# gpustack/llama-box

Measured on AMD Instinct MI355X. Metric: decode tokens/sec (batch-1) + prefill tok/s, Llama-3-8B Q4_K_M, higher is better.
Workload: dtype q4_K/q6_K weights x q8_K activations (int8 dot, f32 accumulate)

## Files before the change

### llama_box_amd/csrc/fattn.hip

```cpp
#include <algorithm>

#include "dev_util.h"
#include "kernels.h"
#include <vector>
#include <algorithm>
#include "kv_dequant.h"

namespace mi355x {

static inline bool fa_g_ok(const int64_t G) {
    static const int g_min = getenv("GGML_MI355X_FA_G_MIN") ? atoi(getenv("GGML_MI355X_FA_G_MIN")) : 1;
    return G >= g_min && G <= 8;
}
static inline int fa_gg(const int64_t G) { return G <= 2 ? 2 : (G <= 4 ? 4 : 8); }

thread_local int g_fa_form = 0;
static inline void fa_form_tail(int tail) { g_fa_form = (g_fa_form & ~(7 << 13)) | (tail << 13); }

struct fa_geom {
    int n_q, n_head, n_kv_head, n_kv, n_splits, has_mask;
    int rec_stride;
    float scale, softcap, max_bias, m0, m1;
    uint32_t n_head_log2;
    unsigned * arrive;
// ... 6 lines not shown
__device__ __forceinline__ float xrow_allsum(const float x) {
    float a = x, b = x;
    asm volatile("s_nop 1\n\tv_permlane16_swap_b32 %0, %1" : "+v"(a), "+v"(b));
    float y = a + b;
    a = y;
    b = y;
    asm volatile("s_nop 1\n\tv_permlane32_swap_b32 %0, %1" : "+v"(a), "+v"(b));
    return a + b;
}

template <int D, int G>
__global__ void __launch_bounds__(256) k_fattn_split(const tdesc q, const tdesc k, const tdesc v, const tdesc mask, const float * __restrict__ sinks,
                                                     const tdesc dst, const fa_geom geo, float * __restrict__ ws) {
    constexpr int LPR = D / 8;
    constexpr int RPW = 64 / LPR;
    constexpr int NG = 4;
    __shared__ float sh[4][G][D + 2];
    const int tid = threadIdx.x, lane = tid & 63, wave = tid >> 6;
    const int sub = lane / LPR, sl = lane % LPR;
    const int split = blockIdx.x, kvh = blockIdx.y;
    const int tok = blockIdx.z % geo.n_q, bat = blockIdx.z / geo.n_q;
    const int per = (geo.n_kv + geo.n_splits - 1) / geo.n_splits;
    const int kv0 = split * per, kv1 = min(geo.n_kv, kv0 + per);
    const int64_t kb = bat / (q.ne[3] / k.ne[3]), vb = bat / (q.ne[3] / v.ne[3]);
    const uint16_t * mp = geo.has_mask ? (const uint16_t *) (mask.data + (int64_t) tok * mask.nb[1] + (int64_t) (bat % mask.ne[3]) * mask.nb[3]) : nullptr;
    const char * kbase = k.data + (int64_t) kvh * k.nb[2] + kb * k.nb[3] + sl * 16;
    const char * vbase = v.data + (int64_t) kvh * v.nb[2] + vb * v.nb[3] + sl * 16;

    uint4 kraw[NG], vraw[NG];
    float mv[NG];
    bool inr[NG];
    int p0 = kv0 + wave * RPW;
#define FA_LOAD_TRIP()                                                        \
    _Pragma("unroll") for (int u = 0; u < NG; ++u) {                         \
        const int p = p0 + u * 4 * RPW + sub;                                 \
        inr[u] = p < kv1;                                                     \
        const int pc = min(p, kv1 - 1);                                       \
        mv[u] = mp ? h2f(mp[pc]) : 0.0f;                                      \
        kraw[u] = *(const uint4 *) (kbase + (int64_t) pc * k.nb[1]);          \
        vraw[u] = *(const uint4 *) (vbase + (int64_t) pc * v.nb[1]);          \
    }
    if (kv0 < kv1) { FA_LOAD_TRIP() }

    float qr[G][8], acc[G][8], m[G], l[G], slope[G];
#pragma unroll
    for (int g = 0; g < G; ++g) {
        const int h = kvh * G + g;
        const float4 * qp = (const float4 *) ((const float *) (q.data + (int64_t) tok * q.nb[1] + (int64_t) h * q.nb[2] + (int64_t) bat * q.nb[3]) + sl * 8);
        const float4 qa = qp[0], qb = qp[1];
        const float qv[8] = {qa.x, qa.y, qa.z, qa.w, qb.x, qb.y, qb.z, qb.w};
#pragma unroll
        for (int i = 0; i < 8; ++i) {
            qr[g][i] = h2f(f2h(qv[i]));
            acc[g][i] = 0.0f;
        }
        m[g] = -INFINITY;
        l[g] = 0.0f;
        slope[g] = geo.max_bias > 0.0f ? ((uint32_t) h < geo.n_head_log2 ? powf(geo.m0, (float) (h + 1)) : powf(geo.m1, (float) (2 * (h - geo.n_head_log2) + 1))) : 1.0f;
    }

    for (; p0 < kv1; p0 += NG * 4 * RPW) {
        float sc[NG][G];
        float vf[NG][8];
#pragma unroll
        for (int u = 0; u < NG; ++u) {
            const uint32_t ku[4] = {kraw[u].x, kraw[u].y, kraw[u].z, kraw[u].w}, vu[4] = {vraw[u].x, vraw[u].y, vraw[u].z, vraw[u].w};
            float kf[8];
#pragma unroll
            for (int i = 0; i < 4; ++i) {
                kf[2 * i] = h2f((uint16_t) (ku[i] & 0xFFFF));
                kf[2 * i + 1] = h2f((uint16_t) (ku[i] >> 16));
                vf[u][2 * i] = h2f((uint16_t) (vu[i] & 0xFFFF));
                vf[u][2 * i + 1] = h2f((uint16_t) (vu[i] >> 16));
            }
#pragma unroll
            for (int g = 0; g < G; ++g) {
                float t = 0.0f;
#pragma unroll
                for (int i = 0; i < 8; ++i) t = fmaf(kf[i], qr[g][i], t);
                if constexpr (LPR == 16) {
                    t = row16_sum(t);
                } else {
                    t += dpp_f32<MI_DPP_QUAD_XOR1>(t);
                    t += dpp_f32<MI_DPP_QUAD_XOR2>(t);
                    t += dpp_f32<MI_DPP_HALF_MIRROR>(t);
                }
                float sv = t * geo.scale;
                if (geo.softcap != 0.0f) sv = geo.softcap * tanhf(sv);
                const float mvs = slope[g] * mv[u];
                sv += mvs;
                sc[u][g] = (inr[u] && !(mvs == -INFINITY)) ? sv : -INFINITY;
            }
        }
        const bool more = p0 + NG * 4 * RPW < kv1;
        if (more) {
            p0 += NG * 4 * RPW;
            FA_LOAD_TRIP()
            p0 -= NG * 4 * RPW;
        }
#pragma unroll
        for (int g = 0; g < G; ++g) {
            float mx = sc[0][g];
#pragma unroll
            for (int u = 1; u < NG; ++u) mx = fmaxf(mx, sc[u][g]);
            mx = wave_max(mx);
            const float mn = fmaxf(m[g], mx);
            if (mn == -INFINITY) continue;
            const float alpha = m[g] == -INFINITY ? 0.0f : expf(m[g] - mn);
            float ps = 0.0f;
#pragma unroll
            for (int i = 0; i < 8; ++i) acc[g][i] *= alpha;
#pragma unroll
            for (int u = 0; u < NG; ++u) {
                const float pe = sc[u][g] == -INFINITY ? 0.0f : expf(sc[u][g] - mn);
                ps += pe;
#pragma unroll
                for (int i = 0; i < 8; ++i) acc[g][i] = fmaf(pe, vf[u][i], acc[g][i]);
            }
            l[g] = l[g] * alpha + ps;
            m[g] = mn;
        }
    }
#undef FA_LOAD_TRIP
#pragma unroll
    for (int g = 0; g < G; ++g) {
        float lt = l[g];
        if constexpr (LPR == 8) lt += dpp_f32<MI_DPP_ROR8>(lt);
        lt = xrow_allsum(lt);
#pragma unroll
        for (int i = 0; i < 8; ++i) {
            float a = acc[g][i];
            if constexpr (LPR == 8) a += dpp_f32<MI_DPP_ROR8>(a);
            acc[g][i] = xrow_allsum(a);
        }
        l[g] = lt;
    }
    if (sub == 0) {
#pragma unroll
        for (int g = 0; g < G; ++g) {
            *(float4 *) &sh[wave][g][sl * 8] = make_float4(acc[g][0], acc[g][1], acc[g][2], acc[g][3]);
            *(float4 *) &sh[wave][g][sl * 8 + 4] = make_float4(acc[g][4], acc[g][5], acc[g][6], acc[g][7]);
            if (sl == 0) {
                sh[wave][g][D] = m[g];
                sh[wave][g][D + 1] = l[g];
            }
        }
    }
    __syncthreads();
    for (int e = tid; e < G * D; e += 256) {
        const int g = e / D, dd = e % D;
        const float m0 = sh[0][g][D], m1 = sh[1][g][D], m2 = sh[2][g][D], m3 = sh[3][g][D];
        const float mt = fmaxf(fmaxf(m0, m1), fmaxf(m2, m3));
        const float c0 = m0 == -INFINITY ? 0.0f : expf(m0 - mt), c1 = m1 == -INFINITY ? 0.0f : expf(m1 - mt);
        const float c2 = m2 == -INFINITY ? 0.0f : expf(m2 - mt), c3 = m3 == -INFINITY ? 0.0f : expf(m3 - mt);
        float a = ((sh[0][g][dd] * c0 + sh[1][g][dd] * c1) + sh[2][g][dd] * c2) + sh[3][g][dd] * c3;
        float lt = ((sh[0][g][D + 1] * c0 + sh[1][g][D + 1] * c1) + sh[2][g][D + 1] * c2) + sh[3][g][D + 1] * c3;
        const int h = kvh * G + g;
        if (geo.n_splits == 1) {
            if (sinks) {
                const float sk = sinks[h];
                const float mn = fmaxf(mt, sk);
                const float c = mt == -INFINITY ? 0.0f : expf(mt - mn);
                a *= c;
                lt = lt * c + expf(sk - mn);
            }
            float * out = (float *) (dst.data + (int64_t) h * dst.nb[1] + (int64_t) tok * dst.nb[2] + (int64_t) bat * dst.nb[3]);
            out[dd] = a * (1.0f / lt);
        } else {
            float * rec = ws + ((((int64_t) bat * geo.n_q + tok) * geo.n_head + h) * geo.n_splits + split) * (D + 2);
            rec[dd] = a;
            if (dd == 0) {
                rec[D] = mt;
                rec[D + 1] = lt;
            }
        }
    }
}

#define MI_DPP_NEWBCAST(n) (0x150 + (n))
typedef _Float16 fa_half2 __attribute__((ext_vector_type(2)));

__device__ __forceinline__ float fa_exp2(const float x) { return __builtin_amdgcn_exp2f(x); }
__device__ __forceinline__ float swap32_pairsum(float x, float y) {
    asm volatile("s_nop 1\n\tv_permlane32_swap_b32 %0, %1" : "+v"(x), "+v"(y));
    return x + y;
}
__device__ __forceinline__ float swap16_pairsum(float c, float d) {
    asm volatile("s_nop 1\n\tv_permlane16_swap_b32 %0, %1" : "+v"(c), "+v"(d));
    return c + d;
}
__device__ __forceinline__ float xrow_allmax(const float x) {
    float a = x, b = x;
    asm volatile("s_nop 1\n\tv_permlane16_swap_b32 %0, %1" : "+v"(a), "+v"(b));
    const float y = fmaxf(a, b);
    a = y;
    b = y;
    asm volatile("s_nop 1\n\tv_permlane32_swap_b32 %0, %1" : "+v"(a), "+v"(b));
    return fmaxf(a, b);
}
__device__ __forceinline__ void st_agent(float * p, const float v) { __hip_atomic_store(p, v, __ATOMIC_RELAXED, __HIP_MEMORY_SCOPE_AGENT); }
__device__ __forceinline__ float ld_agent(const float * p) { return __hip_atomic_load(p, __ATOMIC_RELAXED, __HIP_MEMORY_SCOPE_AGENT); }
__device__ __forceinline__ void st_agent2(float * p, const float a, const float b) {
    const unsigned long long v = (unsigned long long) __builtin_bit_cast(unsigned, a) | ((unsigned long long) __builtin_bit_cast(unsigned, b) << 32);
    __hip_atomic_store((unsigned long long *) p, v, __ATOMIC_RELAXED, __HIP_MEMORY_SCOPE_AGENT);
}
__device__ __forceinline__ float2 ld_agent2(const float * p) {
    const unsigned long long v = __hip_atomic_load((const unsigned long long *) p, __ATOMIC_RELAXED, __HIP_MEMORY_SCOPE_AGENT);
    return make_float2(__builtin_bit_cast(float, (unsigned) v), __builtin_bit_cast(float, (unsigned) (v >> 32)));
}
#define FA_M2_REC 132

__device__ __forceinline__ void fa_merge2(const float * __restrict__ hb, const int h0, const int g_real, const int n_splits, const float * __restrict__ sinks, const tdesc & dst,
                                          const int tok, const int bat, const int n_threads) {
    const int tid = threadIdx.x, lane = tid & 63;
    const int64_t ss = (int64_t) g_real * FA_M2_REC;
#pragma unroll 1
    for (int g = tid >> 7; g < g_real; g += n_threads >> 7) {
        const int dd = tid & 127;
        const float * __restrict__ base = hb + (int64_t) g * FA_M2_REC;
        const float2 ml = ld_agent2(base + (int64_t) min(lane, n_splits - 1) * ss + 128);
        float r[32];
#pragma unroll
        for (int u = 0; u < 32; ++u) r[u] = ld_agent(base + (int64_t) min(u, n_splits - 1) * ss + dd);
        const float ms = lane < n_splits ? ml.x : -INFINITY, ls = lane < n_splits ? ml.y : 0.0f;
        float mn = wave_max(ms);
        float sink_term = 0.0f;
        if (sinks) {
            mn = fmaxf(mn, sinks[h0 + g]);
            sink_term = expf(sinks[h0 + g] - mn);
        }
        const float cs = ms == -INFINITY ? 0.0f : expf(ms - mn);
        const float lt = wave_sum(ls * cs) + sink_term;
        float a = 0.0f;
#pragma unroll
        for (int u = 0; u < 32; ++u) {
            const float c = readlane_f32(cs, u);
            a += c != 0.0f ? r[u] * c : 0.0f;
        }
        float * out = (float *) (dst.data + (int64_t) (h0 + g) * dst.nb[1] + (int64_t) tok * dst.nb[2] + (int64_t) bat * dst.nb[3]);
        out[dd] = a * (1.0f / lt);
    }
}

__device__ __forceinline__ void fa_merge_heads(const float * __restrict__ base0, const int h0, const int g_real, const int n_splits, const float * __restrict__ sinks, const tdesc & dst,
                                               const int tok, const int bat, q8k_dev * __restrict__ q8, float * __restrict__ vals) {
    constexpr int D = 128;
    const int tid = threadIdx.x, lane = tid & 63, wave = tid >> 6;
    if (q8) __syncthreads();
    for (int g = wave; g < g_real; g += 4) {
        const float * __restrict__ base = base0 + (int64_t) g * n_splits * (D + 2);
        const bool has = lane < n_splits;
        const float ms = has ? ld_agent(base + (int64_t) lane * (D + 2) + D) : -INFINITY;
        const float ls = has ? ld_agent(base + (int64_t) lane * (D + 2) + D + 1) : 0.0f;
        float mn = wave_max(ms);
        float sink_term = 0.0f;
        if (sinks) {
            mn = fmaxf(mn, sinks[h0 + g]);
            sink_term = expf(sinks[h0 + g] - mn);
        }
        const float cs = ms == -INFINITY ? 0.0f : expf(ms - mn);
        const float lt = wave_sum(ls * cs) + sink_term;
        float a0 = 0.0f, a1 = 0.0f;
        for (int u0 = 0; u0 < n_splits; u0 += 8) {
            float r0[8], r1[8];
#pragma unroll
            for (int k = 0; k < 8; ++k) {
                const int u = min(u0 + k, n_splits - 1);
                r0[k] = ld_agent(base + (int64_t) u * (D + 2) + lane);
                r1[k] = ld_agent(base + (int64_t) u * (D + 2) + 64 + lane);
            }
#pragma unroll
            for (int k = 0; k < 8; ++k) {
                const float c = u0 + k < n_splits ? readlane_f32(cs, min(u0 + k, 63)) : 0.0f;
                a0 += c != 0.0f ? r0[k] * c : 0.0f;
                a1 += c != 0.0f ? r1[k] * c : 0.0f;
            }
        }
        const float inv = 1.0f / lt;
        if (q8) {
            vals[g * D + lane] = a0 * inv;
            vals[g * D + 64 + lane] = a1 * inv;
        } else {
            float * out = (float *) (dst.data + (int64_t) (h0 + g) * dst.nb[1] + (int64_t) tok * dst.nb[2] + (int64_t) bat * dst.nb[3]);
            out[lane] = a0 * inv;
            out[64 + lane] = a1 * inv;
        }
    }
    if (q8) {
        __syncthreads();
        if (wave < g_real / 2) {
            const float4 t4 = ((const float4 *) (vals + wave * 256))[lane];
            const float t[4] = {t4.x, t4.y, t4.z, t4.w};
            wave_quantize_q8_K(t, lane, q8 + wave);
        }
    }
}

#ifdef FA_STAMP
__device__ unsigned long long g_fa_stamps[1024][8];
#define FA_STAMP_AT(i) { if (WV == 8 && MODE == 0 && threadIdx.x == 0) g_fa_stamps[(blockIdx.y * gridDim.x + blockIdx.x) & 1023][(i)] = __builtin_readcyclecounter(); }
#else
#define FA_STAMP_AT(i)
#endif
template <int G, int MODE, bool Q8, int WV = 4, int KVT = 0, int D = 128>
__global__ void __launch_bounds__(WV * 64) k_fattn_dec128(const tdesc q, const tdesc k, const tdesc v, const tdesc mask, const float * __restrict__ sinks,
                                                      const tdesc dst, const fa_geom geo, float * __restrict__ ws, const int g_real,
                                                      const int * __restrict__ lists, const int list_stride) {
    constexpr bool SKIP = MODE == 1, LIST = MODE == 2;
    constexpr int LPR = D / 8, RPW = 64 / LPR, NG = LPR / G;
    static_assert(D == 128 || (D == 64 && !Q8 && KVT == 0 && G <= 8), "head_dim 64: f16 cache only");
    constexpr float LOG2E = 1.4426950408889634f;
    constexpr int TRIP = NG * WV * RPW;
    constexpr bool BF = KVT == GGML_TYPE_BF16;
    constexpr bool DQ = KVT != 0 && !BF;
    static_assert(WV == 4 || (!Q8 && !DQ && !BF), "the eight-wave forms serve an f16 cache only");
    static_assert(!(Q8 && DQ), "q8_0 has its own integer path");
    constexpr bool FAT = WV == 8 && MODE == 0;
    FA_STAMP_AT(0)
    __shared__ float sh[WV][G][D + 2];
    __shared__ float qv[FAT ? 1 : G * D];
    const int tid = threadIdx.x, lane = tid & 63, wave = tid >> 6;
    const int sub = lane / LPR, sl = lane & (LPR - 1);
    const int ul = sl / G, gl = sl % G;
    const int split = blockIdx.x, kvh = blockIdx.y;
    const int tok = (int) blockIdx.z;
    constexpr int bat = 0;
    const int per = geo.per;
    const int kv0 = LIST ? 0 : min(split * per, geo.n_kv);
    int kv1 = LIST ? 0 : min(geo.n_kv, kv0 + per);
    const int * tl = nullptr;
    int ti = 0, ti1 = 0, cnt = 0;
    bool empty = false;
    int nidx[NG];
    int first = 0;
#define FA_LIST_AHEAD(base)                                                                                         \
    _Pragma("unroll") for (int u = 0; u < NG; ++u) nidx[u] = tl[min((base) + u * (WV * RPW) + wave * RPW + sub, geo.n_kv - 1)];
    if constexpr (LIST) {
        const int * lt = lists + (int64_t) tok * list_stride;
        tl = lt + 1;
        cnt = lt[0];
        first = lt[1];
        if (geo.n_splits == 1) FA_LIST_AHEAD(0)
        const int trips = (cnt + TRIP - 1) / TRIP, share = (trips + geo.n_splits - 1) / geo.n_splits;
        ti = split * share;
        ti1 = min(trips, ti + share);
        if (ti >= ti1) {
            if (geo.n_splits == 1) {
                for (int e = tid; e < g_real * D; e += WV * 64) {
                    float * out = (float *) (dst.data + (int64_t) (kvh * g_real + e / D) * dst.nb[1] + (int64_t) tok * dst.nb[2] + (int64_t) bat * dst.nb[3]);
                    out[e % D] = __builtin_nanf("");
                }
            } else if (tid < g_real) {
                float * rec = ws + ((((int64_t) bat * geo.n_q + tok) * geo.n_head + kvh * g_real + tid) * geo.n_splits + split) * (D + 2);
                if (geo.arrive) { st_agent(rec + D, -INFINITY); st_agent(rec + D + 1, 0.0f); }
                else { rec[D] = -INFINITY; rec[D + 1] = 0.0f; }
            }
            if (geo.n_splits == 1 || !geo.arrive) return;
            empty = true;
        }
        kv1 = cnt;
        if (geo.n_splits != 1 && !empty) FA_LIST_AHEAD(ti * TRIP)
    }
    constexpr int64_t kb = 0, vb = 0, mb = 0;
    if constexpr (SKIP) {
        const uint16_t * mrow = (const uint16_t *) (mask.data + (int64_t) tok * mask.nb[1] + mb * mask.nb[3]);
        bool any = false;
        for (int c0 = kv0; c0 < kv1; c0 += 256) {
            const int pp = c0 + 4 * lane;
            if (pp < kv1) {
                const uint2 w = *(const uint2 *) (mrow + pp);
                any = any || w.x != 0xFC00FC00u || w.y != 0xFC00FC00u;
            }
        }
        if (!__any(any)) {
            if (tid < g_real) {
                float * rec = ws + ((((int64_t) bat * geo.n_q + tok) * geo.n_head + kvh * g_real + tid) * geo.n_splits + split) * (D + 2);
                if (geo.arrive) { st_agent(rec + D, -INFINITY); st_agent(rec + D + 1, 0.0f); }
                else { rec[D] = -INFINITY; rec[D + 1] = 0.0f; }
            }
            if (!geo.arrive) return;
            empty = true;
        }
    }
    if (!empty) {
    const uint16_t * mp = geo.has_mask ? (const uint16_t *) (mask.data + (int64_t) tok * mask.nb[1] + mb * mask.nb[3]) : nullptr;
    const char * kbase = k.data + (int64_t) kvh * k.nb[2] + kb * k.nb[3] + (DQ ? (sl >> 2) * kv_block_bytes_t<KVT>() : Q8 ? (sl >> 2) * 34 + 2 + (sl & 3) * 8 : sl * 16);
    const char * vbase = v.data + (int64_t) kvh * v.nb[2] + vb * v.nb[3] + (DQ ? (sl >> 2) * kv_block_bytes_t<KVT>() : Q8 ? (sl >> 2) * 34 + 2 + (sl & 3) * 8 : sl * 16);

    uint4 kraw[NG], vraw[NG];
    float mvl = 0.0f;
    bool okl = false;
    int p0 = LIST ? ti * TRIP : kv0;
#define FA_LOAD_TRIP()                                                                  \
    {                                                                                   \
        _Pragma("unroll") for (int u = 0; u < NG; ++u) {                               \
            const int pr_ = p0 + u * (WV * RPW) + wave * RPW + sub;                     \
            const int pc = LIST ? (pr_ < kv1 ? nidx[u] : first) : min(pr_, kv1 - 1);    \
            const char * kp_ = kbase + (int64_t) pc * k.nb[1];                          \
            const char * vp_ = vbase + (int64_t) pc * v.nb[1];                          \
            if constexpr (DQ) {   \
                kraw[u] = kv_load_octet_raw_t<KVT>(kp_, sl & 3);                        \
                vraw[u] = kv_load_octet_raw_t<KVT>(vp_, sl & 3);                        \
            } else if constexpr (Q8) {    \
                kraw[u] = make_uint4(ld32_a2(kp_), ld32_a2(kp_ + 4), (uint32_t) ld16(kp_ - 2 - (sl & 3) * 8), 0u);  \
                vraw[u] = make_uint4(ld32_a2(vp_), ld32_a2(vp_ + 4), (uint32_t) ld16(vp_ - 2 - (sl & 3) * 8), 0u);  \
            } else {                                                                    \
                kraw[u] = *(const uint4 *) kp_;                                         \
                vraw[u] = *(const uint4 *) vp_;                                         \
            }                                                                           \
        }                                                                               \
        const int pl = p0 + ul * (WV * RPW) + wave * RPW + sub;                         \
        okl = pl < kv1;                                                                 \
        int plc_ = min(pl, kv1 - 1);                                                    \
        if constexpr (LIST) {                                                           \
            plc_ = nidx[0];                                                             \
            _Pragma("unroll") for (int u = 1; u < NG; ++u) plc_ = ul == u ? nidx[u] : plc_; \
            plc_ = okl ? plc_ : first;                                                  \
        }                                                                               \
        mvl = mp ? h2f(mp[plc_]) : 0.0f;                                                \
        if constexpr (LIST) FA_LIST_AHEAD(p0 + TRIP)                                    \
    }
    uint32_t vis = 0xFFFFFFFFu;
    if constexpr (SKIP) {
        vis = 0;
        const int ntrips = (kv1 - kv0 + TRIP - 1) / TRIP;
        for (int i0 = 0; i0 < ntrips; i0 += 8) {
            uint16_t mraw[8];
#pragma unroll
            for (int i = 0; i < 8; ++i) {
                const int pl = kv0 + (i0 + i) * TRIP + ul * (WV * RPW) + wave * RPW + sub;
                mraw[i] = (i0 + i < ntrips && pl < kv1) ? (mp ? mp[pl] : (uint16_t) 0) : (uint16_t) 0xFC00;
            }
#pragma unroll
            for (int i = 0; i < 8; ++i)
                if (__any(mraw[i] != 0xFC00)) vis |= 1u << (i0 + i);
        }
        if (vis & 1u) FA_LOAD_TRIP()
    } else {
        if (kv0 < kv1) FA_LOAD_TRIP()
    }
    FA_STAMP_AT(1)

    fa_half2 qh[G][4];
    int qq[G][2];
    float dq[G];
    int qsb[G];
    float sq[G];
    float qf[BF ? G : 1][8];
#pragma unroll
    for (int g = 0; g < G; ++g) {
        const int h = kvh * g_real + min(g, g_real - 1);
        const float4 * qp = (const float4 *) ((const float *) (q.data + (int64_t) tok * q.nb[1] + (int64_t) h * q.nb[2] + (int64_t) bat * q.nb[3]) + sl * 8);
        const float4 qa = qp[0], qb = qp[1];
        const float z = g < g_real ? 1.0f : 0.0f;
        if constexpr (BF) {
            const float xv[8] = {qa.x * z, qa.y * z, qa.z * z, qa.w * z, qb.x * z, qb.y * z, qb.z * z, qb.w * z};
#pragma unroll
            for (int i = 0; i < 8; ++i) {
                const uint32_t u = __float_as_uint(xv[i]);
                qf[g][i] = __uint_as_float((u + (0x7fffu + ((u >> 16) & 1u))) & 0xffff0000u);
            }
        } else if constexpr (Q8 || DQ) {
            const float xv[8] = {qa.x * z, qa.y * z, qa.z * z, qa.w * z, qb.x * z, qb.y * z, qb.z * z, qb.w * z};
            float amax = 0.0f;
#pragma unroll
            for (int i = 0; i < 8; ++i) amax = fmaxf(amax, fabsf(xv[i]));
            amax = fmaxf(amax, dpp_f32<MI_DPP_QUAD_XOR1>(amax));
            amax = fmaxf(amax, dpp_f32<MI_DPP_QUAD_XOR2>(amax));
            const float d = amax / 127.0f;
            const float id = d != 0.0f ? 1.0f / d : 0.0f;
            uint32_t w0 = 0, w1 = 0;
#pragma unroll
            for (int i = 0; i < 4; ++i) {
                w0 |= (uint32_t) ((int) roundf(xv[i] * id) & 0xFF) << (8 * i);
                w1 |= (uint32_t) ((int) roundf(xv[4 + i] * id) & 0xFF) << (8 * i);
            }
            qq[g][0] = (int) w0;
            qq[g][1] = (int) w1;
            dq[g] = h2f(f2h(d));
            if constexpr (DQ) {
                int qs_ = dot4((int) w0, 0x01010101, dot4((int) w1, 0x01010101, 0));
                qs_ += dpp_i32<MI_DPP_QUAD_XOR1>(qs_);
                qs_ += dpp_i32<MI_DPP_QUAD_XOR2>(qs_);
                qsb[g] = qs_;
                sq[g] = h2f(f2h((float) qs_ * d));
            }
        } else {
            qh[g][0] = (fa_half2){(_Float16) (qa.x * z), (_Float16) (qa.y * z)};
            qh[g][1] = (fa_half2){(_Float16) (qa.z * z), (_Float16) (qa.w * z)};
            qh[g][2] = (fa_half2){(_Float16) (qb.x * z), (_Float16) (qb.y * z)};
            qh[g][3] = (fa_half2){(_Float16) (qb.z * z), (_Float16) (qb.w * z)};
        }
    }
#ifdef FA_STAMP
    asm volatile("s_waitcnt vmcnt(8)" ::: "memory");
    FA_STAMP_AT(2)
#endif
    float acc[G][8];
#pragma unroll
    for (int g = 0; g < G; ++g)
#pragma unroll
        for (int i = 0; i < 8; ++i) acc[g][i] = 0.0f;
    float m = -INFINITY, l = 0.0f;
    const bool b3 = (sl & 8) != 0, b2 = (sl & 4) != 0, b1 = (sl & 2) != 0, b0 = (sl & 1) != 0;
    const float sc2 = geo.scale * LOG2E;

    for (int trip = 0; LIST ? ti < ti1 : p0 < kv1; ++trip) {
        int p_next = p0 + TRIP;
        if constexpr (LIST) {
            ++ti;
            p_next = ti < ti1 ? ti * TRIP : kv1;
        }
        if constexpr (SKIP) {
            if (!((vis >> trip) & 1u)) {
                if (p_next < kv1 && ((vis >> (trip + 1)) & 1u)) {
                    p0 = p_next;
                    FA_LOAD_TRIP()
                }
                p0 = p_next;
                continue;
            }
        }
        float t[LPR];
        float vf[NG][8];
#pragma unroll
        for (int u = 0; u < NG; ++u) {
            uint32_t ku[4] = {kraw[u].x, kraw[u].y, kraw[u].z, kraw[u].w}, vu[4] = {vraw[u].x, vraw[u].y, vraw[u].z, vraw[u].w};
            if constexpr (DQ) {
                constexpr bool OFFSET = KVT == GGML_TYPE_Q4_1 || KVT == GGML_TYPE_Q5_1;
                uint32_t k0, k1;
                kv_octet_levels_t<KVT, true>(kraw[u], sl & 3, k0, k1);
                const float dk = h2f((uint16_t) (ku[2] & 0xFFFFu));
                const float mk = OFFSET ? h2f((uint16_t) (ku[2] >> 16)) : 0.0f;
                kv_octet_f32_t<KVT>(vraw[u], sl & 3, vf[u]);
#pragma unroll
                for (int g = 0; g < G; ++g) {
                    int isum = dot4((int) k0, qq[g][0], dot4((int) k1, qq[g][1], 0));
                    isum += dpp_i32<MI_DPP_QUAD_XOR1>(isum);
                    isum += dpp_i32<MI_DPP_QUAD_XOR2>(isum);
                    float term;
                    if constexpr (KVT == GGML_TYPE_Q4_0) term = ((float) (isum - 8 * qsb[g]) * dk) * dq[g];
                    else if constexpr (KVT == GGML_TYPE_Q5_0) term = (dk * dq[g]) * (float) (isum - 16 * qsb[g]);
                    else if constexpr (KVT == GGML_TYPE_IQ4_NL) term = (dq[g] * dk) * (float) isum;
                    else term = (dk * dq[g]) * (float) isum + mk * sq[g];
                    t[u * G + g] = (sl & 3) == 0 ? term : 0.0f;
                }
            } else if constexpr (Q8) {
                const float dv = h2f((uint16_t) vu[2]), dk = h2f((uint16_t) ku[2]);
#pragma unroll
                for (int i = 0; i < 4; ++i) {
                    vf[u][i] = (float) (int) (int8_t) (vu[0] >> (8 * i)) * dv;
                    vf[u][4 + i] = (float) (int) (int8_t) (vu[1] >> (8 * i)) * dv;
                }
#pragma unroll
                for (int g = 0; g < G; ++g) {
                    int isum = dot4((int) ku[0], qq[g][0], dot4((int) ku[1], qq[g][1], 0));
                    isum += dpp_i32<MI_DPP_QUAD_XOR1>(isum);
                    isum += dpp_i32<MI_DPP_QUAD_XOR2>(isum);
                    t[u * G + g] = (sl & 3) == 0 ? (float) isum * (dk * dq[g]) : 0.0f;
                }
            } else if constexpr (BF) {
                float kf_[8];
#pragma unroll
                for (int i = 0; i < 4; ++i) {
                    vf[u][2 * i] = __uint_as_float(vu[i] << 16);
                    vf[u][2 * i + 1] = __uint_as_float(vu[i] & 0xffff0000u);
                    kf_[2 * i] = __uint_as_float(ku[i] << 16);
                    kf_[2 * i + 1] = __uint_as_float(ku[i] & 0xffff0000u);
                }
#pragma unroll
                for (int g = 0; g < G; ++g) {
                    float d = 0.0f;
#pragma unroll
                    for (int i = 0; i < 8; ++i) d = __builtin_fmaf(kf_[i], qf[g][i], d);
                    t[u * G + g] = d;
                }
            } else {
#pragma unroll
                for (int i = 0; i < 4; ++i) {
                    vf[u][2 * i] = h2f((uint16_t) (vu[i] & 0xFFFF));
                    vf[u][2 * i + 1] = h2f((uint16_t) (vu[i] >> 16));
                }
#pragma unroll
                for (int g = 0; g < G; ++g) {
                    float d = 0.0f;
#pragma unroll
                    for (int i = 0; i < 4; ++i) d = __builtin_amdgcn_fdot2(__builtin_bit_cast(fa_half2, ku[i]), qh[g][i], d, false);
                    t[u * G + g] = d;
                }
            }
        }
#ifdef FA_STAMP
        if (trip == 0) { asm volatile("" :: "v"(t[0]), "v"(t[15])); FA_STAMP_AT(3) }
#endif
        const bool more = p_next < kv1 && (!SKIP || ((vis >> (trip + 1)) & 1u));
        const float mv_cur = mvl;
        const bool ok_cur = okl;
        p0 = p_next;
        if (more) FA_LOAD_TRIP()
        float w8[8], w4[4], w2[2];
#pragma unroll
        for (int j = 0; j < 8; ++j) {
            if constexpr (LPR == 16) {
                const float keep = b3 ? t[j + 8] : t[j], send = b3 ? t[j] : t[j + 8];
                w8[j] = keep + dpp_f32<MI_DPP_ROR8>(send);
            } else {
                w8[j] = t[j];
            }
        }
#pragma unroll
        for (int j = 0; j < 4; ++j) {
            const float keep = b2 ? w8[j + 4] : w8[j], send = b2 ? w8[j] : w8[j + 4];
            w4[j] = keep + dpp_f32<MI_DPP_HALF_MIRROR>(send);
        }
#pragma unroll
        for (int j = 0; j < 2; ++j) {
            const float keep = b1 ? w4[j + 2] : w4[j], send = b1 ? w4[j] : w4[j + 2];
            w2[j] = keep + dpp_f32<MI_DPP_QUAD_XOR2>(send);
        }
        float sv;
        {
            const float keep = b0 ? w2[1] : w2[0], send = b0 ? w2[0] : w2[1];
            sv = keep + dpp_f32<MI_DPP_QUAD_XOR1>(send);
        }
        sv = (ok_cur && !(mv_cur == -INFINITY)) ? fmaf(sv, sc2, mv_cur * LOG2E) : -INFINITY;
        float mx = sv;
        if constexpr (G <= 2) mx = fmaxf(mx, dpp_f32<MI_DPP_ROR2>(mx));
        if constexpr (G <= 4) mx = fmaxf(mx, dpp_f32<MI_DPP_ROR4>(mx));
        mx = fmaxf(mx, dpp_f32<MI_DPP_ROR8>(mx));
        mx = xrow_allmax(mx);
        const float mn = fmaxf(m, mx);
        const float mref = mn == -INFINITY ? 0.0f : mn;
        const float alpha = fa_exp2(m - mref);
        const float pe = fa_exp2(sv - mref);
        l = l * alpha + pe;
        m = mn;
#define FA_HEAD(g)                                                                          \
    if constexpr ((g) < G) {                                                                \
        const float ag_ = dpp_f32<MI_DPP_NEWBCAST((g))>(alpha);                             \
        _Pragma("unroll") for (int i = 0; i < 8; ++i) acc[(g)][i] *= ag_;                  \
    }
        FA_HEAD(0) FA_HEAD(1) FA_HEAD(2) FA_HEAD(3) FA_HEAD(4) FA_HEAD(5) FA_HEAD(6) FA_HEAD(7)
#undef FA_HEAD
#define FA_PAIR(j)                                                                          \
    {                                                                                       \
        const float pj_ = dpp_f32<MI_DPP_NEWBCAST((j))>(pe);                                \
        _Pragma("unroll") for (int i = 0; i < 8; ++i) acc[(j) % G][i] = fmaf(pj_, vf[(j) / G][i], acc[(j) % G][i]); \
    }
#define FA_PAIR8(j)                                                                         \
    {                                                                                       \
        const float pa_ = dpp_f32<MI_DPP_NEWBCAST((j))>(pe), pb_ = dpp_f32<MI_DPP_NEWBCAST((j) + 8)>(pe); \
        const float pj_ = (lane & 8) ? pb_ : pa_;                                           \
        _Pragma("unroll") for (int i = 0; i < 8; ++i) acc[(j) % G][i] = fmaf(pj_, vf[(j) / G][i], acc[(j) % G][i]); \
    }
        if constexpr (LPR == 16) {
            FA_PAIR(0) FA_PAIR(1) FA_PAIR(2) FA_PAIR(3) FA_PAIR(4) FA_PAIR(5) FA_PAIR(6) FA_PAIR(7)
            FA_PAIR(8) FA_PAIR(9) FA_PAIR(10) FA_PAIR(11) FA_PAIR(12) FA_PAIR(13) FA_PAIR(14) FA_PAIR(15)
        } else {
            FA_PAIR8(0) FA_PAIR8(1) FA_PAIR8(2) FA_PAIR8(3) FA_PAIR8(4) FA_PAIR8(5) FA_PAIR8(6) FA_PAIR8(7)
        }
#undef FA_PAIR8
#undef FA_PAIR
    }
#undef FA_LOAD_TRIP
#undef FA_LIST_AHEAD
#ifdef FA_STAMP
    asm volatile("" :: "v"(acc[0][0]), "v"(acc[G - 1][7]));
    FA_STAMP_AT(4)
#endif
    if constexpr (G <= 2) l += dpp_f32<MI_DPP_ROR2>(l);
    if constexpr (G <= 4) l += dpp_f32<MI_DPP_ROR4>(l);
    l += dpp_f32<MI_DPP_ROR8>(l);
    l = xrow_allsum(l);
    if constexpr (LPR == 8) {
#pragma unroll
        for (int g = 0; g < G; ++g)
#pragma unroll
            for (int i = 0; i < 8; ++i) acc[g][i] += dpp_f32<MI_DPP_ROR8>(acc[g][i]);
    }
#pragma unroll
    for (int kk = 0; kk < 2 * G; ++kk) {
        const int g = (4 * kk) / 8, i0 = (4 * kk) % 8;
        const float y1 = swap32_pairsum(acc[g][i0], acc[g][i0 + 2]);
        const float y2 = swap32_pairsum(acc[g][i0 + 1], acc[g][i0 + 3]);
        const float z = swap16_pairsum(y1, y2);
        sh[wave][g][sl * 8 + i0 + (lane >> 4)] = z;
    }
    if (sub == 0 && ul == 0) {
        sh[wave][gl][D] = m;
        sh[wave][gl][D + 1] = l;
    }
    __syncthreads();
    FA_STAMP_AT(5)
    for (int e = tid; e < g_real * D; e += WV * 64) {
        const int g = e / D, dd = e % D;
        float mt, a, lt;
        if constexpr (WV == 4) {
            const float m0 = sh[0][g][D], m1 = sh[1][g][D], m2 = sh[2][g][D], m3 = sh[3][g][D];
            mt = fmaxf(fmaxf(m0, m1), fmaxf(m2, m3));
            const float mref = mt == -INFINITY ? 0.0f : mt;
            const float c0 = fa_exp2(m0 - mref), c1 = fa_exp2(m1 - mref), c2 = fa_exp2(m2 - mref), c3 = fa_exp2(m3 - mref);
            a = ((sh[0][g][dd] * c0 + sh[1][g][dd] * c1) + sh[2][g][dd] * c2) + sh[3][g][dd] * c3;
            lt = ((sh[0][g][D + 1] * c0 + sh[1][g][D + 1] * c1) + sh[2][g][D + 1] * c2) + sh[3][g][D + 1] * c3;
        } else {
            mt = sh[0][g][D];
#pragma unroll
            for (int w = 1; w < WV; ++w) mt = fmaxf(mt, sh[w][g][D]);
            const float mref = mt == -INFINITY ? 0.0f : mt;
            a = 0.0f;
            lt = 0.0f;
#pragma unroll
            for (int w = 0; w < WV; ++w) {
                const float c = fa_exp2(sh[w][g][D] - mref);
                a += sh[w][g][dd] * c;
                lt += sh[w][g][D + 1] * c;
            }
        }
        const int h = kvh * g_real + g;
        const float mt_e = mt * (1.0f / LOG2E);
        if (geo.n_splits == 1 && (!FAT || geo.rec_stride == D + 2)) {
            if (sinks) {
                const float sk = sinks[h];
                const float mn = fmaxf(mt_e, sk);
                const float c = mt == -INFINITY ? 0.0f : expf(mt_e - mn);
                a *= c;
                lt = lt * c + expf(sk - mn);
            }
            if (!FAT && geo.q8) qv[g * D + dd] = a * (1.0f / lt);
            else {
                float * out = (float *) (dst.data + (int64_t) h * dst.nb[1] + (int64_t) tok * dst.nb[2] + (int64_t) bat * dst.nb[3]);
                out[dd] = a * (1.0f / lt);
            }
        } else {
            float * rec = ws + ((((int64_t) bat * geo.n_q + tok) * geo.n_head + h) * geo.n_splits + split) * geo.rec_stride;
            if (geo.merge2) {
                float * r2 = ws + (((((int64_t) bat * geo.n_q + tok) * geo.n_kv_head + kvh) * geo.n_splits + split) * g_real + g) * FA_M2_REC;
                const float nb = dpp_f32<0xF5>(a);
                if ((dd & 1) == 0) st_agent2(r2 + dd, a, nb);
                if (dd == 0) st_agent2(r2 + D, mt_e, lt);
            } else if (WV == 4 && geo.arrive) {
                st_agent(rec + dd, a);
                if (dd == 0) { st_agent(rec + D, mt_e); st_agent(rec + D + 1, lt); }
            } else {
                rec[dd] = a;
                if (dd == 0) {
                    rec[D] = mt_e;
                    rec[D + 1] = lt;
                }
            }
        }
    }
    FA_STAMP_AT(6)
    }
    if constexpr (D == 128)
    if (geo.merge2) {
        __shared__ int s_last2;
        asm volatile("s_waitcnt vmcnt(0)" ::: "memory");
        __syncthreads();
        if (tid == 0) {
            unsigned * cnt_p = geo.arrive + ((int64_t) bat * geo.n_q + tok) * geo.n_kv_head + kvh;
            const unsigned old = __hip_atomic_fetch_add(cnt_p, 1u, __ATOMIC_RELAXED, __HIP_MEMORY_SCOPE_AGENT);
            s_last2 = old == (unsigned) geo.n_splits - 1u;
            if (s_last2) __hip_atomic_store(cnt_p, 0u, __ATOMIC_RELAXED, __HIP_MEMORY_SCOPE_AGENT);
        }
        __syncthreads();
        if (!s_last2) return;
        fa_merge2(ws + ((((int64_t) bat * geo.n_q + tok) * geo.n_kv_head + kvh) * geo.n_splits) * (int64_t) (g_real * FA_M2_REC), kvh * g_real, g_real, geo.n_splits, sinks, dst, tok, bat,
                  WV * 64);
        return;
    }
    if constexpr (!FAT && D == 128) {
        if (geo.n_splits == 1 && geo.q8) {
            __syncthreads();
            if (wave < g_real / 2) {
                const float4 t4 = ((const float4 *) (qv + wave * 256))[lane];
                const float t[4] = {t4.x, t4.y, t4.z, t4.w};
                wave_quantize_q8_K(t, lane, (q8k_dev *) geo.q8 + ((int64_t) bat * geo.n_q + tok) * (geo.n_head * D / 256) + (kvh * g_real) / 2 + wave);
            }
        }
        if constexpr (WV == 4)
        if (geo.n_splits > 1 && geo.arrive) {
            __shared__ int s_last;
            asm volatile("s_waitcnt vmcnt(0)" ::: "memory");
            __syncthreads();
            if (tid == 0) {
                unsigned * cnt_p = geo.arrive + ((int64_t) bat * geo.n_q + tok) * geo.n_kv_head + kvh;
                const unsigned old = __hip_atomic_fetch_add(cnt_p, 1u, __ATOMIC_RELAXED, __HIP_MEMORY_SCOPE_AGENT);
                s_last = old == (unsigned) geo.n_splits - 1u;
                if (s_last) __hip_atomic_store(cnt_p, 0u, __ATOMIC_RELAXED, __HIP_MEMORY_SCOPE_AGENT);
            }
            __syncthreads();
            if (!s_last) return;
            fa_merge_heads((const float *) ws + (((int64_t) bat * geo.n_q + tok) * geo.n_head + kvh * g_real) * geo.n_splits * (D + 2), kvh * g_real, g_real, geo.n_splits, sinks, dst,
                           tok, bat, geo.q8 ? (q8k_dev *) geo.q8 + ((int64_t) bat * geo.n_q + tok) * (geo.n_head * D / 256) + (kvh * g_real) / 2 : nullptr, &sh[0][0][0]);
        }
    }
}

template <int D, bool Q8OUT = false> __global__ void __launch_bounds__(Q8OUT ? 256 : D) k_fattn_combine(const float * __restrict__ ws, const float * __restrict__ sinks, const tdesc dst, const fa_geom geo,
                                                                                                 q8k_dev * __restrict__ q8 = nullptr) {
    const int h = Q8OUT ? (int) blockIdx.x * (256 / D) + (int) threadIdx.x / D : (int) blockIdx.x, tok = blockIdx.y, bat = blockIdx.z, dd = threadIdx.x % D, lane = threadIdx.x & 63;
    const float * __restrict__ base = ws + (((int64_t) bat * geo.n_q + tok) * geo.n_head + h) * geo.n_splits * (D + 2);
    const bool has = lane < geo.n_splits;
    const float ms = has ? base[(int64_t) lane * (D + 2) + D] : -INFINITY;
    const float ls = has ? base[(int64_t) lane * (D + 2) + D + 1] : 0.0f;
    float r0[32], r1[32];
#pragma unroll
    for (int u = 0; u < 32; ++u) r0[u] = base[(int64_t) min(u, geo.n_splits - 1) * (D + 2) + dd];
    const bool second = geo.n_splits > 32;
    if (second) {
#pragma unroll
        for (int u = 0; u < 32; ++u) r1[u] = base[(int64_t) min(32 + u, geo.n_splits - 1) * (D + 2) + dd];
    }
    float mn = wave_max(ms);
    float sink_term = 0.0f;
    if (sinks) {
        mn = fmaxf(mn, sinks[h]);
        sink_term = expf(sinks[h] - mn);
    }
    const float cs = ms == -INFINITY ? 0.0f : expf(ms - mn);
    const float lt = wave_sum(ls * cs) + sink_term;
    float a = 0.0f;
#pragma unroll
    for (int u = 0; u < 32; ++u) {
        const float c = readlane_f32(cs, u);
        a += c != 0.0f ? r0[u] * c : 0.0f;
    }
    if (second) {
#pragma unroll
        for (int u = 0; u < 32; ++u) {
            const float c = readlane_f32(cs, 32 + u);
            a += c != 0.0f ? r1[u] * c : 0.0f;
        }
    }
    if constexpr (Q8OUT) {
        __shared__ float vals[256];
        vals[threadIdx.x] = a * (1.0f / lt);
        __syncthreads();
        if (threadIdx.x < 64) {
            const float4 t4 = ((const float4 *) vals)[lane];
            const float t[4] = {t4.x, t4.y, t4.z, t4.w};
            wave_quantize_q8_K(t, lane, q8 + ((int64_t) bat * geo.n_q + tok) * (geo.n_head * D / 256) + blockIdx.x);
        }
    } else {
        float * out = (float *) (dst.data + (int64_t) h * dst.nb[1] + (int64_t) tok * dst.nb[2] + (int64_t) bat * dst.nb[3]);
        out[dd] = a * (1.0f / lt);
    }
}

template <int D, int S, bool Q8OUT = false>
__global__ void __launch_bounds__(256) k_fattn_combine_rows(const float * __restrict__ ws, const tdesc dst, const fa_geom geo, const int n_rows, q8k_dev * __restrict__ q8 = nullptr) {
    constexpr int CPR = D / 4;
    constexpr int RPB = 256 / CPR;
    const int r = (int) blockIdx.x * RPB + (int) threadIdx.x / CPR, j = (int) threadIdx.x % CPR;
    if (r >= n_rows) return;
    const int h = r % geo.n_head, tok = (r / geo.n_head) % geo.n_q, bat = r / (geo.n_head * geo.n_q);
    const float * __restrict__ base = ws + (int64_t) r * geo.n_splits * (D + 2);
    float4 v[S];
    float2 ml[S];
#pragma unroll
    for (int u = 0; u < S; ++u) {
        const int uu = min(u, geo.n_splits - 1);
        const float2 v0 = *(const float2 *) (base + (int64_t) uu * (D + 2) + 4 * j), v1 = *(const float2 *) (base + (int64_t) uu * (D + 2) + 4 * j + 2);
        v[u] = make_float4(v0.x, v0.y, v1.x, v1.y);
        ml[u] = *(const float2 *) (base + (int64_t) uu * (D + 2) + D);
    }
    float mn = -INFINITY;
#pragma unroll
    for (int u = 0; u < S; ++u) mn = fmaxf(mn, u < geo.n_splits ? ml[u].x : -INFINITY);
    float lt = 0.0f;
    float4 a = make_float4(0.0f, 0.0f, 0.0f, 0.0f);
#pragma unroll
    for (int u = 0; u < S; ++u) {
        const float c = (u < geo.n_splits && ml[u].x != -INFINITY) ? expf(ml[u].x - mn) : 0.0f;
        lt += (u < geo.n_splits ? ml[u].y : 0.0f) * c;
        a.x += c != 0.0f ? v[u].x * c : 0.0f;
        a.y += c != 0.0f ? v[u].y * c : 0.0f;
        a.z += c != 0.0f ? v[u].z * c : 0.0f;
        a.w += c != 0.0f ? v[u].w * c : 0.0f;
    }
    const float inv = 1.0f / lt;
    if constexpr (Q8OUT) {
        static_assert(D == 128, "two heads of 128 = one block");
        const float t[4] = {a.x * inv, a.y * inv, a.z * inv, a.w * inv};
        wave_quantize_q8_K(t, (int) threadIdx.x & 63, q8 + (r >> 1));
    } else {
        float * out = (float *) (dst.data + (int64_t) h * dst.nb[1] + (int64_t) tok * dst.nb[2] + (int64_t) bat * dst.nb[3]);
        *(float4 *) (out + 4 * j) = make_float4(a.x * inv, a.y * inv, a.z * inv, a.w * inv);
    }
}

bool fattn_combine_rows_applies(int D, int64_t n_q, int64_t n_head, int64_t n_batch, int n_splits, const float * sinks) {
    static const bool rows_on = !getenv("GGML_MI355X_FA_COMBINE_ROWS") || atoi(getenv("GGML_MI355X_FA_COMBINE_ROWS")) != 0;
    const int64_t n_rows = n_batch * n_q * n_head;
    return rows_on && !sinks && D == 128 && n_splits >= 2 && n_splits <= 8 && n_rows >= 2048 && n_rows < (1 << 30);
}
void launch_flash_attn_combine(hipStream_t s, int D, const float * ws, const float * sinks, const tdesc & dst, int n_q, int n_head, int n_batch, int n_splits, void * q8_out) {
    fa_geom geo{};
    geo.n_q = n_q;
    geo.n_head = n_head;
    geo.n_splits = n_splits;
    const int64_t n_rows = (int64_t) n_batch * n_q * n_head;
    if (fattn_combine_rows_applies(D, n_q, n_head, n_batch, n_splits, sinks) && (((uintptr_t) ws) & 7) == 0 &&
        (q8_out ? (n_head % 2) == 0 : ((dst.nb[1] % 16) == 0 && (dst.nb[2] % 16) == 0 && (dst.nb[3] % 16) == 0 && (((uintptr_t) dst.data) & 15) == 0))) {
        const unsigned blocks = (unsigned) ((n_rows + 7) / 8);
        fa_form_tail(FA_FORM_TAIL_COMBINE_ROWS);
        if (q8_out) {
            if (n_splits <= 4) hipLaunchKernelGGL((k_fattn_combine_rows<128, 4, true>), dim3(blocks), dim3(256), 0, s, ws, dst, geo, (int) n_rows, (q8k_dev *) q8_out);
            else hipLaunchKernelGGL((k_fattn_combine_rows<128, 8, true>), dim3(blocks), dim3(256), 0, s, ws, dst, geo, (int) n_rows, (q8k_dev *) q8_out);
        } else {
            if (n_splits <= 4) hipLaunchKernelGGL((k_fattn_combine_rows<128, 4>), dim3(blocks), dim3(256), 0, s, ws, dst, geo, (int) n_rows, (q8k_dev *) nullptr);
            else hipLaunchKernelGGL((k_fattn_combine_rows<128, 8>), dim3(blocks), dim3(256), 0, s, ws, dst, geo, (int) n_rows, (q8k_dev *) nullptr);
        }
        return;
    }
    dim3 g2((unsigned) n_head, (unsigned) n_q, (unsigned) n_batch);
    fa_form_tail(FA_FORM_TAIL_COMBINE);
    if (q8_out && D == 128) {
        hipLaunchKernelGGL((k_fattn_combine<128, true>), dim3((unsigned) (n_head / 2), (unsigned) n_q, (unsigned) n_batch), dim3(256), 0, s, ws, sinks, dst, geo, (q8k_dev *) q8_out);
        return;
    }
    if (D == 128) hipLaunchKernelGGL((k_fattn_combine<128>), g2, dim3(128), 0, s, ws, sinks, dst, geo);
    else hipLaunchKernelGGL((k_fattn_combine<64>), g2, dim3(64), 0, s, ws, sinks, dst, geo);
}

bool fattn_prefers_lists(const tdesc & q, const tdesc * mask, int mask_sparse) {
    static const bool on = !getenv("GGML_MI355X_FA_SPARSE_LISTS") || atoi(getenv("GGML_MI355X_FA_SPARSE_LISTS")) != 0;
    return on && mask != nullptr && q.ne[1] >= fattn_mma_min_q() && q.ne[1] <= 256 && mask_sparse != 0;
}
int fattn_pick_splits(const tdesc & q, const tdesc & k, const tdesc * mask, int mask_sparse) {
    if (q.ne[1] >= fattn_mma_min_q() && (k.ne[0] == 64 || k.ne[0] == 128) && !fattn_prefers_lists(q, mask, mask_sparse)) return fattn_mma_pick_splits(q, k);
    const int64_t n_kv = k.ne[1];
    if (q.ne[1] > 1 && (k.ne[0] == 128 || (k.ne[0] == 64 && k.type == GGML_TYPE_F16 && k.ne[2] > 0 && q.ne[2] % k.ne[2] == 0 && fa_g_ok(q.ne[2] / k.ne[2]))) && q.ne[3] == 1) {
        const int64_t groups = k.ne[2] * q.ne[1];
        const int64_t trips = std::max<int64_t>(1, (n_kv / q.ne[1] + 63) / 64);
        const int64_t by_len = (trips + 7) / 8, by_occ = std::min<int64_t>(trips, (256 + groups - 1) / groups);
        return (int) std::max<int64_t>(1, std::min<int64_t>(16, std::max(by_len, by_occ)));
    }
    if (q.ne[1] > 1) {
        const int64_t by_len = (n_kv + 255) / 256;
        return (int) std::max<int64_t>(1, std::min<int64_t>(64, std::min<int64_t>(by_len, std::max<int64_t>(1, n_kv / 64))));
    }
    const int64_t groups = k.ne[2] * q.ne[1] * q.ne[3];
    int64_t want = (768 + groups - 1) / groups;
    const int64_t max_by_len = std::max<int64_t>(1, n_kv / 86);
    want = std::max<int64_t>(1, std::min<int64_t>(want, std::min<int64_t>(max_by_len, 64)));
    if (k.type == GGML_TYPE_F16 && q.ne[1] == 1 && want * groups > 256) want = std::max<int64_t>(1, 256 / groups);
    return (int) want;
}
static size_t fattn_partials_bytes(const tdesc & q, const tdesc & v, int n_splits) {
    if (n_splits <= 1) return 0;
    return ((size_t) (q.ne[1] * q.ne[3] * q.ne[2]) * (size_t) std::max(n_splits, 16) * (size_t) (v.ne[0] + 4) * sizeof(float) + 255) & ~(size_t) 255;
}
int fattn_fat_splits(const tdesc & q, const tdesc & k, const tdesc * mask, const float * sinks, const fattn_params & p) {
    if (q.ne[1] != 1 || q.ne[3] != 1 || k.ne[0] != 128 || k.ne[3] != 1 || p.kv_type != GGML_TYPE_F16 || sinks || p.logit_softcap != 0.0f || p.max_bias != 0.0f) return 0;
    if (q.ne[2] % k.ne[2] != 0 || (q.ne[2] % 2) != 0) return 0;
    const int64_t G = q.ne[2] / k.ne[2];
    if (!fa_g_ok(G) || (q.nb[1] % 16) != 0 || (q.nb[2] % 16) != 0 || ((uintptr_t) q.data & 15) != 0) return 0;
    if (mask && (mask->type != GGML_TYPE_F16)) return 0;
    const int64_t trip = 32 * (16 / fa_gg(G));
    const int64_t trips = (k.ne[1] + trip - 1) / trip;
    int64_t splits = std::min<int64_t>(12, trips);
    const int64_t per = (trips + splits - 1) / splits;
    splits = (trips + per - 1) / per;
    return (int) splits;
}
static bool fattn_q8_via_f16(const tdesc & q, int kv_type) { return kv_type == GGML_TYPE_Q8_0 && q.ne[1] >= fattn_mma_min_q(); }
size_t fattn_workspace_bytes(const tdesc & q, const tdesc & k, const tdesc & v, int n_splits, int kv_type) {
// ... 320 lines not shown
```

Measured before the change: 572.7.

## Skip dead KV row groups in decode attention, add nontemporal KV loads and late mask

The decode flash-attention kernel now works out, per wave, how many rows of the current trip are live. It skips KV loads, list prefetches, QK dot products and PV accumulation for row groups past the end of the KV range. The eight-wave f16 path reads K/V with nontemporal loads, and the mask value is kept as a raw half and converted only when used. A waitcnt placed before issuing the next trip's loads changes how memory ops overlap. The extra branches and waitcnt could serialize loads or add control overhead, and attention is only a small part of batch-1 decode time.

```diff
diff --git a/llama_box_amd/csrc/fattn.hip b/llama_box_amd/csrc/fattn.hip
--- a/llama_box_amd/csrc/fattn.hip
+++ b/llama_box_amd/csrc/fattn.hip
@@ -332,6 +332,17 @@
 #else
 #define FA_STAMP_AT(i)
 #endif
+#ifndef FA_KV_NT
+#define FA_KV_NT 1
+#endif
+#ifndef FA_MASK_LATE
+#define FA_MASK_LATE 1
+#endif
+typedef uint32_t fa_u32x4 __attribute__((ext_vector_type(4)));
+static __device__ __forceinline__ uint4 fa_ld_nt16(const char * p) {
+    const fa_u32x4 r = __builtin_nontemporal_load((const fa_u32x4 *) p);
+    return make_uint4(r.x, r.y, r.z, r.w);
+}
 template <int G, int MODE, bool Q8, int WV = 4, int KVT = 0, int D = 128>
 __global__ void __launch_bounds__(WV * 64) k_fattn_dec128(const tdesc q, const tdesc k, const tdesc v, const tdesc mask, const float * __restrict__ sinks,
                                                       const tdesc dst, const fa_geom geo, float * __restrict__ ws, const int g_real,
@@ -361,16 +372,20 @@
     const int * tl = nullptr;
     int ti = 0, ti1 = 0, cnt = 0;
     bool empty = false;
-    int nidx[NG];
+    int nidx[NG] = {};
     int first = 0;
+    const int wrow = __builtin_amdgcn_readfirstlane(wave) * RPW;
+#define FA_LIVE(base, u) (SKIP || (base) + (u) * (WV * RPW) + wrow < kv1)
+#define FA_LIST_AHEAD_ALL(base)                                                                                     \
+    _Pragma("unroll") for (int u = 0; u < NG; ++u) nidx[u] = tl[min((base) + u * (WV * RPW) + wave * RPW + sub, geo.n_kv - 1)];
 #define FA_LIST_AHEAD(base)                                                                                         \
-    _Pragma("unroll") for (int u = 0; u < NG; ++u) nidx[u] = tl[min((base) + u * (WV * RPW) + wave * RPW + sub, geo.n_kv - 1)];
+    _Pragma("unroll") for (int u = 0; u < NG; ++u) if (FA_LIVE(base, u)) nidx[u] = tl[min((base) + u * (WV * RPW) + wave * RPW + sub, geo.n_kv - 1)];
     if constexpr (LIST) {
         const int * lt = lists + (int64_t) tok * list_stride;
         tl = lt + 1;
         cnt = lt[0];
         first = lt[1];
-        if (geo.n_splits == 1) FA_LIST_AHEAD(0)
+        if (geo.n_splits == 1) FA_LIST_AHEAD_ALL(0)
         const int trips = (cnt + TRIP - 1) / TRIP, share = (trips + geo.n_splits - 1) / geo.n_splits;
         ti = split * share;
         ti1 = min(trips, ti + share);
@@ -419,11 +434,12 @@
 
     uint4 kraw[NG], vraw[NG];
     float mvl = 0.0f;
+    uint16_t mrl = 0;
     bool okl = false;
     int p0 = LIST ? ti * TRIP : kv0;
 #define FA_LOAD_TRIP()                                                                  \
     {                                                                                   \
-        _Pragma("unroll") for (int u = 0; u < NG; ++u) {                               \
+        _Pragma("unroll") for (int u = 0; u < NG; ++u) if (FA_LIVE(p0, u)) {           \
             const int pr_ = p0 + u * (WV * RPW) + wave * RPW + sub;                     \
             const int pc = LIST ? (pr_ < kv1 ? nidx[u] : first) : min(pr_, kv1 - 1);    \
             const char * kp_ = kbase + (int64_t) pc * k.nb[1];                          \
@@ -434,12 +450,15 @@
             } else if constexpr (Q8) {    \
                 kraw[u] = make_uint4(ld32_a2(kp_), ld32_a2(kp_ + 4), (uint32_t) ld16(kp_ - 2 - (sl & 3) * 8), 0u);  \
                 vraw[u] = make_uint4(ld32_a2(vp_), ld32_a2(vp_ + 4), (uint32_t) ld16(vp_ - 2 - (sl & 3) * 8), 0u);  \
+            } else if constexpr (FA_KV_NT != 0 && FAT && !BF) {   \
+                kraw[u] = fa_ld_nt16(kp_);                                              \
+                vraw[u] = fa_ld_nt16(vp_);                                              \
             } else {                                                                    \
                 kraw[u] = *(const uint4 *) kp_;                                         \
                 vraw[u] = *(const uint4 *) vp_;                                         \
             }                                                                           \
         }                                                                               \
-        const int pl = p0 + ul * (WV * RPW) + wave * RPW + sub;                         \
+        const int pl = p0 + ul * (WV * RPW) + wave * RPW + sub;                        \
         okl = pl < kv1;                                                                 \
         int plc_ = min(pl, kv1 - 1);                                                    \
         if constexpr (LIST) {                                                           \
@@ -447,7 +466,8 @@
             _Pragma("unroll") for (int u = 1; u < NG; ++u) plc_ = ul == u ? nidx[u] : plc_; \
             plc_ = okl ? plc_ : first;                                                  \
         }                                                                               \
-        mvl = mp ? h2f(mp[plc_]) : 0.0f;                                                \
+        if constexpr (FA_MASK_LATE != 0) mrl = mp ? mp[plc_] : (uint16_t) 0;            \
+        else mvl = mp ? h2f(mp[plc_]) : 0.0f;                                           \
         if constexpr (LIST) FA_LIST_AHEAD(p0 + TRIP)                                    \
     }
     uint32_t vis = 0xFFFFFFFFu;
@@ -553,8 +573,14 @@
         }
         float t[LPR];
         float vf[NG][8];
+        const int rem = SKIP ? NG * WV * RPW : kv1 - p0 - wrow;
 #pragma unroll
         for (int u = 0; u < NG; ++u) {
+            if (u * (WV * RPW) >= rem) {
+#pragma unroll
+                for (int g = 0; g < G; ++g) t[u * G + g] = 0.0f;
+                continue;
+            }
             uint32_t ku[4] = {kraw[u].x, kraw[u].y, kraw[u].z, kraw[u].w}, vu[4] = {vraw[u].x, vraw[u].y, vraw[u].z, vraw[u].w};
             if constexpr (DQ) {
                 constexpr bool OFFSET = KVT == GGML_TYPE_Q4_1 || KVT == GGML_TYPE_Q5_1;
@@ -624,10 +650,13 @@
         if (trip == 0) { asm volatile("" :: "v"(t[0]), "v"(t[15])); FA_STAMP_AT(3) }
 #endif
         const bool more = p_next < kv1 && (!SKIP || ((vis >> (trip + 1)) & 1u));
-        const float mv_cur = mvl;
+        const float mv_cur = FA_MASK_LATE != 0 ? h2f(mrl) : mvl;
         const bool ok_cur = okl;
         p0 = p_next;
-        if (more) FA_LOAD_TRIP()
+        if (more) {
+            if constexpr (!SKIP) __builtin_amdgcn_s_waitcnt(0x0F70);
+            FA_LOAD_TRIP()
+        }
         float w8[8], w4[4], w2[2];
 #pragma unroll
         for (int j = 0; j < 8; ++j) {
@@ -683,17 +712,23 @@
         const float pj_ = (lane & 8) ? pb_ : pa_;                                           \
         _Pragma("unroll") for (int i = 0; i < 8; ++i) acc[(j) % G][i] = fmaf(pj_, vf[(j) / G][i], acc[(j) % G][i]); \
     }
-        if constexpr (LPR == 16) {
-            FA_PAIR(0) FA_PAIR(1) FA_PAIR(2) FA_PAIR(3) FA_PAIR(4) FA_PAIR(5) FA_PAIR(6) FA_PAIR(7)
-            FA_PAIR(8) FA_PAIR(9) FA_PAIR(10) FA_PAIR(11) FA_PAIR(12) FA_PAIR(13) FA_PAIR(14) FA_PAIR(15)
-        } else {
-            FA_PAIR8(0) FA_PAIR8(1) FA_PAIR8(2) FA_PAIR8(3) FA_PAIR8(4) FA_PAIR8(5) FA_PAIR8(6) FA_PAIR8(7)
-        }
+#define FA_PAIR_G(u, g) if constexpr ((g) < G) { if constexpr (LPR == 16) FA_PAIR((u) * G + (g)) else FA_PAIR8((u) * G + (g)) }
+#define FA_GROUP(u)                                                                         \
+    if constexpr ((u) < NG) {                                                               \
+        if ((u) * (WV * RPW) < rem) {                                                       \
+            FA_PAIR_G(u, 0) FA_PAIR_G(u, 1) FA_PAIR_G(u, 2) FA_PAIR_G(u, 3) FA_PAIR_G(u, 4) FA_PAIR_G(u, 5) FA_PAIR_G(u, 6) FA_PAIR_G(u, 7) \
+        }                                                                                   \
+    }
+        FA_GROUP(0) FA_GROUP(1) FA_GROUP(2) FA_GROUP(3) FA_GROUP(4) FA_GROUP(5) FA_GROUP(6) FA_GROUP(7)
+#undef FA_GROUP
+#undef FA_PAIR_G
 #undef FA_PAIR8
 #undef FA_PAIR
     }
 #undef FA_LOAD_TRIP
 #undef FA_LIST_AHEAD
+#undef FA_LIST_AHEAD_ALL
+#undef FA_LIVE
 #ifdef FA_STAMP
     asm volatile("" :: "v"(acc[0][0]), "v"(acc[G - 1][7]));
     FA_STAMP_AT(4)
```

New measurement: 589.9 (median of 6 runs). 1.03x the previous value.
